# xiangli0608/Creating-2D-laser-slam-from-scratch

Measured on AMD Instinct MI355X. Metric: scan-matches/sec (1081-beam vs 2000x2000 grid), higher is better.
Workload: dtype u8

## Files before the change

### creating-2d-laser-slam-from-scratch_amd/csrc/scan_matcher.hip

```cpp
#include <algorithm>
#include <atomic>
#include <chrono>
#include <cmath>
#include <cstdlib>
#include <cstring>
#include <type_traits>
#include <vector>

#include "common.hpp"
#include "karto_math.hpp"

using namespace lslam;

#if defined(LSLAM_EXP_SERIAL_PRIO)
#define LSLAM_SERIAL_BEGIN() __builtin_amdgcn_s_setprio(3)
#define LSLAM_SERIAL_END() __builtin_amdgcn_s_setprio(0)
#else
#define LSLAM_SERIAL_BEGIN()
#define LSLAM_SERIAL_END()
#endif

namespace {

LSLAM_STAMP_TABLE(g_sm_stamps)
// ... 140 lines not shown
  };
  auto cell_y = [&](int j) {
    double y = start_y + (uint32_t)j * pc.res_y;
    double npy = center[1] + y;
    return world_to_grid(npy, g.off_y, g.scale) + g.border;
  };
  const int stx0 = pc.nx > 1 ? cell_x(1) - cell_x(0) : want_step;
  const int sty0 = pc.ny > 1 ? cell_y(1) - cell_y(0) : want_step;
  bool out_of_range = false, uneven_x = false, uneven_y = false;
  Lattice& L = lat[s];
  for (int i = lane; i < kMaxLattice; i += 64) {
    int cx = 0, cy = 0;
    if (i < pc.nx) {
      cx = cell_x(i);
      out_of_range |= cx < 0 || cx >= g.width;
      if (i >= 1) uneven_x |= cx - cell_x(i - 1) != stx0;
    }
    if (i < pc.ny) {
      cy = cell_y(i);
      out_of_range |= cy < 0 || cy >= g.height;
      if (i >= 1) uneven_y |= cy - cell_y(i - 1) != sty0;
    }
    L.gx[i] = cx;
    L.gy[i] = cy;
  }
  for (int a = lane; a < pc.na; a += 64) {
    const double angle = (center[2] - pc.ang_off) + (uint32_t)a * pc.ang_res;
    cossin[(size_t)s * kMaxAngles + a] = make_double2(cos(angle), sin(angle));
  }
  const int status = __any(out_of_range) ? LSLAM_ERR_INDEX_OUT_OF_RANGE : 0;
  const int stx = __any(uneven_x) ? 0 : stx0, sty = __any(uneven_y) ? 0 : sty0;
  if (lane == 0) {
    L.center[0] = center[0]; L.center[1] = center[1]; L.center[2] = center[2];
    L.step_x = stx;
    L.step_y = sty;
    L.status = status;
    L.active = active;
  }
}

__global__ void __launch_bounds__(64)
k_pass_setup(int S, Geom g, PassCfg pc, const double* __restrict__ poses, const CoarseOut* __restrict__ coarse,
             Lattice* __restrict__ lat, double2* __restrict__ cossin, int want_step) {
  const int s = blockIdx.x;
  if (s >= S) return;
  double center[3];
  int active = 1;
  if (pc.mode == 0) {
    center[0] = poses[3 * s]; center[1] = poses[3 * s + 1]; center[2] = poses[3 * s + 2];
  } else if (pc.mode == 1) {
    center[0] = poses[3 * s]; center[1] = poses[3 * s + 1]; center[2] = poses[3 * s + 2];
    active = coarse[s].expand && coarse[s].status == 0;
  } else {
    center[0] = coarse[s].mean[0]; center[1] = coarse[s].mean[1]; center[2] = coarse[s].mean[2];
    active = coarse[s].status == 0;
  }
  pass_setup_wave(s, threadIdx.x, g, pc, center, active, lat, cossin, want_step);
}

__global__ void __launch_bounds__(256)
k_deinterleave(const uint8_t* __restrict__ grid, uint8_t* __restrict__ f0, uint8_t* __restrict__ f1, int n8) {
  int t = blockIdx.x * blockDim.x + threadIdx.x;
  if (t >= n8) return;
  uint2 v = ((const uint2*)grid)[t];
  uint32_t e = (v.x & 0xFFu) | ((v.x >> 8) & 0xFF00u) | ((v.y & 0xFFu) << 16) | ((v.y << 8) & 0xFF000000u);
  uint32_t o = ((v.x >> 8) & 0xFFu) | ((v.x >> 16) & 0xFF00u) | ((v.y << 8) & 0xFF0000u) | (v.y & 0xFF000000u);
  ((uint32_t*)f0)[t] = e;
  ((uint32_t*)f1)[t] = o;
}

__global__ void __launch_bounds__(256)
k_tile_planes(const uint8_t* __restrict__ grid, int stride, int data_size, uint32_t* __restrict__ tiles,
              int tile_tx, int tile_rows) {
  const size_t d = (size_t)blockIdx.x * blockDim.x + threadIdx.x;
  const size_t per_class = (size_t)tile_tx * tile_rows * 8;
  if (d >= 4 * per_class) return;
  const int cls = (int)(d / per_class);
  const size_t rem = d - (size_t)cls * per_class;
  const int c4 = (int)(rem & 7);
  const size_t t = rem >> 3;
  const int row = (int)(t % tile_rows), tx = (int)(t / tile_rows);
  const int q = cls >> 1, ry = cls & 1;
  const long long y = (long long)(2 * row + ry) - kTileYOff;
  const long long m = y * (stride / 2) + 16 * tx + 4 * c4;
  uint32_t v = 0;
#pragma unroll
  for (int k = 0; k < 4; k++) {
    const long long idx = 2 * (m + k) + q;
    if (m + k >= 0 && idx < data_size) v |= (uint32_t)grid[idx] << (8 * k);
  }
  tiles[kTilePad / 4 + d] = v;
}

constexpr int kOccWinMax = 63;

__global__ void __launch_bounds__(256)
k_nonzero_bits(const uint8_t* __restrict__ grid, int data_size, uint32_t* __restrict__ nz, int n_words) {
  int w = blockIdx.x * blockDim.x + threadIdx.x;
  if (w >= n_words) return;
  uint32_t bits = 0;
  const long long f0 = (long long)w * 32;
  if (f0 + 32 <= data_size) {
    const uint4* p = (const uint4*)(grid + f0);
    uint4 a = p[0], b = p[1];
    const uint32_t v[8] = {a.x, a.y, a.z, a.w, b.x, b.y, b.z, b.w};
#pragma unroll
    for (int k = 0; k < 8; k++) {
      uint32_t d = v[k];
      bits |= ((d & 0xFFu) ? 1u : 0u) << (4 * k);
      bits |= ((d & 0xFF00u) ? 1u : 0u) << (4 * k + 1);
      bits |= ((d & 0xFF0000u) ? 1u : 0u) << (4 * k + 2);
      bits |= ((d & 0xFF000000u) ? 1u : 0u) << (4 * k + 3);
    }
  } else {
    for (int k = 0; k < 32; k++)
      if (f0 + k < data_size && grid[f0 + k] != 0) bits |= 1u << k;
  }
  nz[w] = bits;
}

__global__ void __launch_bounds__(256)
k_row_occupancy(const uint32_t* __restrict__ nz, int n_words, int stride, int height, int win,
                uint32_t* __restrict__ occ_t, int words_per_half) {
  int x = blockIdx.x * blockDim.x + threadIdx.x;
  int wq = blockIdx.y;
  if (x >= stride || wq >= 2 * words_per_half) return;
  const int E = wq / words_per_half, w2 = wq - E * words_per_half;
  const unsigned long long wmask = (1ull << win) - 1ull;
  uint32_t bits = 0;
  for (int b = 0; b < 32; b++) {
    int y = 2 * (w2 * 32 + b) + E - 1;
    if (y > height) break;
    long long f = (long long)x + (long long)y * stride;
    long long w0 = f >> 5;
    int sh = (int)(f & 31);
    unsigned long long lo = 0, hi = 0;
    if (w0 >= 0 && w0 < n_words) lo = nz[w0];
    if (w0 + 1 >= 0 && w0 + 1 < n_words) lo |= (unsigned long long)nz[w0 + 1] << 32;
    if (w0 + 2 >= 0 && w0 + 2 < n_words) hi = nz[w0 + 2];
    unsigned long long window = (lo >> sh) | (sh ? (hi << (64 - sh)) : 0ull);
    if (window & wmask) bits |= 1u << b;
  }
  occ_t[(size_t)x * (2 * words_per_half) + wq] = bits;
}

__global__ void __launch_bounds__(256)
k_occ_pairs(const uint32_t* __restrict__ occ_t, int stride, int words_per_half, uint2* __restrict__ pairs) {
  const int x = blockIdx.x * blockDim.x + threadIdx.x;
  const int ew = blockIdx.y;
  if (x >= stride) return;
  const int w = ew % words_per_half, E = ew / words_per_half;
  const uint32_t* col = occ_t + (size_t)x * (2 * words_per_half) + ew;
  pairs[((size_t)w * stride + x) * 2 + E] = make_uint2(col[0], w + 1 < words_per_half ? col[1] : 0u);
}

__device__ __forceinline__ uint32_t wave_sum(uint32_t v) {
  v += (uint32_t)__builtin_amdgcn_mov_dpp((int)v, 0xB1, 0xF, 0xF, true);
  v += (uint32_t)__builtin_amdgcn_mov_dpp((int)v, 0x4E, 0xF, 0xF, true);
  v += (uint32_t)__builtin_amdgcn_mov_dpp((int)v, 0x141, 0xF, 0xF, true);
  v += (uint32_t)__builtin_amdgcn_mov_dpp((int)v, 0x140, 0xF, 0xF, true);
  return (uint32_t)__builtin_amdgcn_readlane((int)v, 0) + (uint32_t)__builtin_amdgcn_readlane((int)v, 16) +
         (uint32_t)__builtin_amdgcn_readlane((int)v, 32) + (uint32_t)__builtin_amdgcn_readlane((int)v, 48);
}

constexpr int kPatchDw = 1536;
__device__ __forceinline__ uint32_t wave_min_u32(uint32_t v) {
  v = min(v, (uint32_t)__builtin_amdgcn_mov_dpp((int)v, 0xB1, 0xF, 0xF, true));
  v = min(v, (uint32_t)__builtin_amdgcn_mov_dpp((int)v, 0x4E, 0xF, 0xF, true));
  v = min(v, (uint32_t)__builtin_amdgcn_mov_dpp((int)v, 0x141, 0xF, 0xF, true));
  v = min(v, (uint32_t)__builtin_amdgcn_mov_dpp((int)v, 0x140, 0xF, 0xF, true));
  return min(min((uint32_t)__builtin_amdgcn_readlane((int)v, 0), (uint32_t)__builtin_amdgcn_readlane((int)v, 16)),
             min((uint32_t)__builtin_amdgcn_readlane((int)v, 32), (uint32_t)__builtin_amdgcn_readlane((int)v, 48)));
}
__device__ __forceinline__ uint32_t wave_max_u32(uint32_t v) { return ~wave_min_u32(~v); }
__device__ __forceinline__ void first_valid_min(int* s_first, bool valid, int i) {
  const unsigned long long m = __ballot(valid);
  if (m && (int)(threadIdx.x & 63) == __ffsll((long long)m) - 1) atomicMin(s_first, i);
}

constexpr int kRowsQueue = 256;
struct RowsLds {
  uint32_t (*red)[8];
  int2* queue;
  uint16_t* ambq;
  uint32_t (*patch)[kPatchDw];
  unsigned long long* ambm;
};
template <bool SOLO>
__device__ __forceinline__ void wsync() {
  if constexpr (SOLO) {
    __syncthreads();
  } else {
    __builtin_amdgcn_fence(__ATOMIC_ACQ_REL, "wavefront");
    __builtin_amdgcn_wave_barrier();
  }
}

template <int NXD, int NYC, bool TILED, bool STATS, bool LDSB, bool SOLO, bool OUT_LDS = !SOLO>
__device__ __forceinline__ void resp_rows_wave(
    const int s, const int a, const int slice, const uint8_t* __restrict__ src0, const uint8_t* __restrict__ src1, int step,
    int limit, const Geom& g, const PassCfg& pc, const Lattice* __restrict__ lat, const double2* __restrict__ cossin,
    const double2* __restrict__ local, int32_t* __restrict__ resp, size_t resp_stride, int beam_slices,
    const uint2* __restrict__ occ_t, int occ_wpc, int tile_rows, uint32_t tile_class_bytes,
    unsigned long long* __restrict__ stats, const RowsLds lds, int32_t* lds_out) {
  constexpr int NW = NXD * NYC * 2;
  constexpr bool EST = TILED;
  constexpr int kQueue = kRowsQueue;
  static_assert(NYC <= 16 && 2 * (NYC - 1) < 32, "row mask / occupancy window width");
  static_assert(SOLO || (!STATS && !LDSB), "multi-wave blocks run the production variants only");
  static_assert(!(SOLO && OUT_LDS), "a lone wave writes its numerators to global memory");
  uint32_t (*const red)[8] = lds.red;
  int2* const queue = lds.queue;
  [[maybe_unused]] uint16_t* const ambq = lds.ambq;
  [[maybe_unused]] uint32_t (*const patch)[kPatchDw] = lds.patch;
  [[maybe_unused]] unsigned long long* const ambm = lds.ambm;
  LSLAM_PHASE_CLOCK(pck);
  const Lattice& L = lat[s];
  if (!L.active || L.status != 0 || L.step_x != step || L.step_y != step) return;

  const double2 cs = cossin[(size_t)s * kMaxAngles + a];
  const double cosine = cs.x, sine = cs.y;
  auto uniform = [](float v) { return __int_as_float(__builtin_amdgcn_readfirstlane(__float_as_int(v))); };
  const float cos_sc = uniform((float)cosine * (float)g.scale), sin_sc = uniform((float)sine * (float)g.scale);
  const int X0 = L.gx[0], Y0 = L.gy[0];
  const double2* lp = local + (size_t)s * g.n_beams;
  const int ncand = pc.nx * pc.ny;
  const int shift = step == 2 ? 1 : 0;
  const int bstride = 64 * beam_slices;
  const uint8_t* zbase = TILED ? src0 : src0 - kRowZero;
  const uint32_t plane_delta = TILED ? 0u : (uint32_t)(src1 - src0);
  const uint32_t strip_bytes = (uint32_t)tile_rows * 32u;
  [[maybe_unused]] const int occ_wph = occ_wpc >> 1;

  LSLAM_PHASE_MARK(pck, 0);
  for (int j0 = 0; j0 < pc.ny; j0 += NYC) {
#if defined(LSLAM_EXP_NO_PEEL)
    constexpr bool PEEL = false;
#else
    constexpr bool PEEL = EST;
#endif
    uint32_t acc[NYC][NXD][2];
    if constexpr (!PEEL) {
#pragma unroll
      for (int j = 0; j < NYC; j++)
#pragma unroll
        for (int k = 0; k < NXD; k++) acc[j][k][0] = acc[j][k][1] = 0u;
    }
    uint32_t all_lanes = ~0u;
    asm volatile("" : "+s"(all_lanes));
    const int lane = (int)__builtin_amdgcn_mbcnt_hi(all_lanes, __builtin_amdgcn_mbcnt_lo(all_lanes, 0u));

    auto drain_as = [&](auto first_drain, int head, int cnt) {
      constexpr bool FIRST = decltype(first_drain)::value;
      const int2 e = lane < cnt ? queue[(head + lane) & (kQueue - 1)] : make_int2(0, 0);
      const uint32_t sh = (uint32_t)e.x & 3u;
      const uint32_t sel_e = 0x0C020C00u + sh * 0x00010001u;
      const uint32_t sel_o = 0x0C030C01u + sh * 0x00010001u;
      uint32_t wv[NYC][NXD + 1];
      if constexpr (TILED) {
        const uint32_t xa = (uint32_t)e.x & 0x7FFCu, yy = (uint32_t)e.x >> 16;
        const uint32_t base_off = (uint32_t)kTilePad + (((uint32_t)e.x >> 15) & 1u) * 2u * tile_class_bytes +
                                  (yy & 1u) * tile_class_bytes + (xa >> 4) * strip_bytes + (yy >> 1) * 32u +
                                  (xa & 15u);
#pragma unroll
        for (int j = 0; j < NYC; j++) {
          const uint32_t off = base_off & (uint32_t)__builtin_amdgcn_sbfe(e.y, j, 1);
          __builtin_memcpy(wv[j], __builtin_assume_aligned(zbase + (size_t)off + 32 * j, 4), 4 * (NXD + 1));
        }
      } else {
        bool staged = false;
        if constexpr (LDSB) {
          const uint32_t rowmask = (uint32_t)e.y & ((1u << NYC) - 1u);
          const bool on = lane < cnt && rowmask != 0u && e.x >= 0;
          const uint32_t cur0 = ((uint32_t)e.x & ~3u) + (uint32_t)kRowZero;
          const uint32_t ry = cur0 / (uint32_t)g.stride, cx = cur0 - ry * (uint32_t)g.stride;
          const bool p1 = e.y < 0;
          const bool bad = lane < cnt && rowmask != 0u && e.x < 0;
          uint32_t W[2], Hh[2], cmin[2], rmin[2];
          bool fit = !__any(bad);
#pragma unroll
          for (int q = 0; q < 2; q++) {
            const bool mine = on && (p1 == (q == 1));
            cmin[q] = wave_min_u32(mine ? cx : 0xFFFFFFFFu);
            rmin[q] = wave_min_u32(mine ? ry : 0xFFFFFFFFu);
            const uint32_t cmax = wave_max_u32(mine ? cx + 4u * (NXD + 1) : 0u), rmax = wave_max_u32(mine ? ry + NYC : 0u);
            W[q] = cmax > cmin[q] ? (cmax - cmin[q]) >> 2 : 0u;
            Hh[q] = rmax > rmin[q] ? rmax - rmin[q] : 0u;
            fit = fit && W[q] * Hh[q] <= (uint32_t)kPatchDw && W[q] < 65536u && Hh[q] < 65536u;
          }
          if constexpr (STATS)
            if (lane == 0 && stats) atomicAdd(&stats[fit ? 5 : 6], 1ull);
          if (fit) {
            staged = true;
            const uint32_t limit_bytes = (uint32_t)limit + (uint32_t)kRowZero;
#pragma unroll
            for (int q = 0; q < 2; q++) {
              const uint32_t total = W[q] * Hh[q];
              if (total == 0u) continue;
              const uint32_t inv = 0xFFFFFFFFu / W[q] + 1u;
              for (uint32_t idx = (uint32_t)lane; idx < total; idx += 64u) {
                const uint32_t r = __umulhi(idx, inv), c = idx - r * W[q];
                const uint32_t off = (rmin[q] + r) * (uint32_t)g.stride + cmin[q] + 4u * c;
                uint32_t v = 0u;
                if (off + 4u <= limit_bytes + 64u) v = *(const uint32_t*)(zbase + (size_t)off + (q ? plane_delta : 0u));
                patch[q][idx] = v;
              }
// ... 277 lines not shown
        const double2 p = p_next;
        p_next = lp[min(b + bstride, g.n_beams - 1)];
        const bool valid = (int)(b < g.n_beams) & (int)!isnan(p.x) & (int)!isnan(p.y);
        if constexpr (STATS) st_beams += valid ? 1u : 0u;
        int gx = 0, gy = 0;
        bool small = true;
        if (valid) exact_cell(p, gx, gy, small);
        emit(std::false_type{}, b, valid, small, gx, gy, 0, false, true, 0, 0);
      }
    }
    if (qcount > 0) drain(qhead, qcount);
    wsync<SOLO>();
    LSLAM_PHASE_MARK(pck, 1);
    if constexpr (STATS) {
      const uint32_t t0 = wave_sum(st_rows), t1 = wave_sum(st_live), t2 = wave_sum(st_beams), t3 = wave_sum(st_queued);
      if (lane == 0 && stats) {
        atomicAdd(&stats[0], (unsigned long long)t0);
        atomicAdd(&stats[1], (unsigned long long)t1);
        atomicAdd(&stats[2], (unsigned long long)t2);
        atomicAdd(&stats[3], (unsigned long long)t3);
      }
    }

#pragma unroll
    for (int j = 0; j < NYC; j++)
#pragma unroll
      for (int k = 0; k < NXD; k++)
#pragma unroll
        for (int q = 0; q < 2; q++) {
          uint32_t v = acc[j][k][q];
          v += (uint32_t)__builtin_amdgcn_mov_dpp((int)v, 0xB1, 0xF, 0xF, true);
          v += (uint32_t)__builtin_amdgcn_mov_dpp((int)v, 0x4E, 0xF, 0xF, true);
#if defined(LSLAM_EXP_NO_FUSED_DPP)
          v += (uint32_t)__builtin_amdgcn_mov_dpp((int)v, 0x141, 0xF, 0xF, true);
#else
          asm("s_nop 1\n\tv_add_u32_dpp %0, %0, %0 row_half_mirror row_mask:0xf bank_mask:0xf bound_ctrl:1" : "+v"(v));
#endif
          if ((lane & 7) == 0) red[(j * NXD + k) * 2 + q][lane >> 3] = v;
        }
    wsync<SOLO>();
    for (int idx = lane; idx < NW; idx += 64) {
      uint32_t lo = 0, hi = 0;
#pragma unroll
      for (int k = 0; k < 8; k++) {
        const uint32_t v = red[idx][k];
        lo += v & 0xFFFFu;
        hi += v >> 16;
      }
      const int par2 = idx & 1, jk = idx >> 1;
      const int j = j0 + jk / NXD, i = 4 * (jk % NXD) + par2;
      if (j < pc.ny) {
        if constexpr (OUT_LDS) {
          int32_t* o = lds_out + a * ncand + j * pc.nx + i;
          if (i < pc.nx) o[0] = (int32_t)lo;
          if (i + 2 < pc.nx) o[2] = (int32_t)hi;
        } else {
          int32_t* o = resp + (size_t)s * resp_stride + (size_t)a * ncand + (size_t)j * pc.nx + i;
          if (beam_slices == 1) {
            if (i < pc.nx) o[0] = (int32_t)lo;
            if (i + 2 < pc.nx) o[2] = (int32_t)hi;
          } else {
            if (i < pc.nx) atomicAdd(o, (int32_t)lo);
            if (i + 2 < pc.nx) atomicAdd(o + 2, (int32_t)hi);
          }
        }
      }
    }
    wsync<SOLO>();
    LSLAM_PHASE_MARK(pck, 2);
  }
  if constexpr (SOLO) LSLAM_PHASE_FLUSH(pck, g_sm_stamps, 5, (unsigned)blockIdx.x, (threadIdx.x & 63) == 0);
}

template <int NXD, int NYC, bool TILED, bool STATS = false, bool LDSB = false>
__global__ void __launch_bounds__(64) __attribute__((amdgpu_waves_per_eu(4, 8)))
k_resp_rows(const uint8_t* __restrict__ src0, const uint8_t* __restrict__ src1, int step, int limit, Geom g,
            PassCfg pc, const Lattice* __restrict__ lat, const double2* __restrict__ cossin,
            const double2* __restrict__ local, int32_t* __restrict__ resp, size_t resp_stride, int beam_slices,
            int S, const uint2* __restrict__ occ_t, int occ_wpc, int tile_rows, uint32_t tile_class_bytes,
            unsigned long long* __restrict__ stats) {
  constexpr int NW = NXD * NYC * 2;
  __shared__ __align__(16) uint32_t red[NW][8];
  __shared__ int2 queue[kRowsQueue];
  __shared__ uint16_t ambq[TILED ? 64 * kMaxBeamsPerLane : 1];
  __shared__ uint32_t patch[LDSB ? 2 : 1][LDSB ? kPatchDw : 1];
  int w = blockIdx.x;
  const int slice = w % beam_slices;
  w /= beam_slices;
  const int xcd = w & 7, r = w >> 3;
  const int s = (r / pc.na) * 8 + xcd;
  const int a = r % pc.na;
  if (s >= S) return;
  resp_rows_wave<NXD, NYC, TILED, STATS, LDSB, true>(s, a, slice, src0, src1, step, limit, g, pc, lat, cossin, local, resp,
                                                     resp_stride, beam_slices, occ_t, occ_wpc, tile_rows, tile_class_bytes,
                                                     stats, RowsLds{red, queue, ambq, (uint32_t (*)[kPatchDw])patch, nullptr},
                                                     nullptr);
}

template <int NXD>
constexpr int rows_wave_area() {
  return (NXD == 3 ? 3 * 11 * 2 * 8 * 4 : 4 * 8 * 2 * 8 * 4) > kRowsQueue * 8
             ? (NXD == 3 ? 3 * 11 * 2 * 8 * 4 : 4 * 8 * 2 * 8 * 4) + kMaxBeamsPerLane * 8
             : kRowsQueue * 8 + kMaxBeamsPerLane * 8;
}
template <int NXD, int NYC, int WAVES>
__global__ void __launch_bounds__(64 * WAVES) __attribute__((amdgpu_waves_per_eu(4, 8)))
k_resp_rows_mw(const uint8_t* __restrict__ ptiles, int limit, Geom g, PassCfg pc, const Lattice* __restrict__ lat,
               const double2* __restrict__ cossin, const double2* __restrict__ local, int32_t* __restrict__ resp,
               size_t resp_stride, int S, const uint2* __restrict__ occ_t, int occ_wpc, int tile_rows,
               uint32_t tile_class_bytes) {
  constexpr int kArea = rows_wave_area<NXD>();
  __shared__ __align__(16) unsigned char areas[WAVES * kArea];
  const int wave = (int)threadIdx.x >> 6;
  const int groups = (pc.na + WAVES - 1) / WAVES;
  const int w = blockIdx.x;
  const int xcd = w & 7, r = w >> 3;
  const int s = (r / groups) * 8 + xcd;
  const int a = (r % groups) * WAVES + wave;
  if (s >= S || a >= pc.na) return;
  unsigned char* wa = areas + wave * kArea;
  const RowsLds lds{(uint32_t (*)[8])wa, (int2*)wa, nullptr, nullptr, (unsigned long long*)(wa + (kArea - kMaxBeamsPerLane * 8))};
  resp_rows_wave<NXD, NYC, true, false, false, false, false>(s, a, 0, ptiles, ptiles, 2, limit, g, pc, lat, cossin, local, resp,
                                                             resp_stride, 1, occ_t, occ_wpc, tile_rows, tile_class_bytes,
                                                             (unsigned long long*)nullptr, lds, (int32_t*)nullptr);
}

__host__ __device__ __forceinline__ size_t tile4_slot(int ux, int uy, int cols4) {
  return ((size_t)((uy >> 1) * cols4 + (ux >> 2)) << 3) | (size_t)(((uy & 1) << 2) | (ux & 3));
}
constexpr int kTileYPad = 4;

__global__ void __launch_bounds__(256)
k_tile4(const uint8_t* __restrict__ grid, int stride, int data_size, uint4* __restrict__ tiles, int tile_cols,
        int tile_rows) {
  const int ux = blockIdx.x * blockDim.x + threadIdx.x, uy = blockIdx.y;
  if (ux >= tile_cols || uy >= tile_rows) return;
  const long long idx0 = (long long)(2 * uy - kTileYPad) * stride + 2 * ux;
  uint32_t w[4];
#pragma unroll
  for (int r = 0; r < 4; r++) {
    const long long i = idx0 + (long long)r * stride;
    uint32_t lo = 0, hi = 0;
    if (i >= 0 && i < data_size) lo = *reinterpret_cast<const uint16_t*>(grid + i);
    if (i + 2 >= 0 && i + 2 < data_size) hi = *reinterpret_cast<const uint16_t*>(grid + i + 2);
    w[r] = lo | (hi << 16);
  }
  tiles[tile4_slot(ux, uy, (tile_cols + 3) / 4)] = make_uint4(w[0], w[1], w[2], w[3]);
}

#if !defined(LSLAM_TUNE_TILE3_MIN)
#define LSLAM_TUNE_TILE3_MIN 1536
#endif
constexpr int kTile3ManyAngles = 3, kTile3ManyMinScans = LSLAM_TUNE_TILE3_MIN;
template <int kTile3Angles>
__device__ __forceinline__ void resp_tile3_wave(const int s, const int a0, const int lane, const uint4* __restrict__ tiles,
                                                int tile_cols, const Geom& g, const PassCfg& pc,
                                                const Lattice* __restrict__ lat, const double2* __restrict__ cossin,
                                                const double2* __restrict__ local, int32_t* r_scan) {
  const Lattice& L = lat[s];
  if (!L.active || L.status != 0 || L.step_x != 1 || L.step_y != 1) return;

  double cosine[kTile3Angles], sine[kTile3Angles];
  float cos_sc[kTile3Angles], sin_sc[kTile3Angles];
  bool angle_on[kTile3Angles];
#pragma unroll
  for (int q = 0; q < kTile3Angles; q++) {
    angle_on[q] = a0 + q < pc.na;
    const double2 cs = cossin[(size_t)s * kMaxAngles + min(a0 + q, pc.na - 1)];
    cosine[q] = cs.x, sine[q] = cs.y;
    cos_sc[q] = (float)cs.x * (float)g.scale, sin_sc[q] = (float)cs.y * (float)g.scale;
  }
  const int X0 = L.gx[0], Y0 = L.gy[0];
  const int B0 = X0 + Y0 * g.stride;
  const int cols4 = (tile_cols + 3) / 4;
  const double2* lp = local + (size_t)s * g.n_beams;
  uint32_t e0[kTile3Angles], e1[kTile3Angles], e2[kTile3Angles], o01[kTile3Angles], o2[kTile3Angles];
#pragma unroll
  for (int q = 0; q < kTile3Angles; q++) e0[q] = e1[q] = e2[q] = o01[q] = o2[q] = 0u;
  auto block_of = [&](const double2& p, float x32, float y32, int q, uint32_t& off, uint32_t& dx) {
    const float fx = __builtin_fmaf(cos_sc[q], x32, -(sin_sc[q] * y32)), fy = __builtin_fmaf(sin_sc[q], x32, cos_sc[q] * y32);
    const float rx = __builtin_rintf(fx), ry = __builtin_rintf(fy);
    const float reach = fabsf(fx) + fabsf(fy);
    const float lim = (0.5f - 1e-6f) - reach * (14.2f / 16777216.0f);
    int gx = (int)rx, gy = (int)ry;
    bool small = true;
    double vx = 0.0, vy = 0.0;
    if (!((int)(fabsf(fx - rx) < lim) & (int)(fabsf(fy - ry) < lim) & (int)(reach < 32000.0f))) {
      const double ox = cosine[q] * p.x - sine[q] * p.y, oy = sine[q] * p.x + cosine[q] * p.y;
      vx = ((ox + g.off_x) - g.off_x) * g.scale, vy = ((oy + g.off_y) - g.off_y) * g.scale;
      const double ax = fabs(vx) + 0.5, ay = fabs(vy) + 0.5;
      gx = (int)copysign(ax, vx), gy = (int)copysign(ay, vy);
      small = fmax(ax, ay) < 32768.0;
    }
    int x, y;
    bool ok;
    if (small) {
      x = X0 + gx, y = Y0 + gy;
      if ((uint32_t)x >= (uint32_t)g.stride) {
        const int base = B0 + gx + __mul24(gy, g.stride);
        y = base >= 0 ? base / g.stride : -((-base + g.stride - 1) / g.stride);
        x = base - y * g.stride;
      }
      ok = y >= -3 && y < g.height;
    } else {
      const int gxl = kround_i32(vx), gyl = kround_i32(vy);
      const long long base = (long long)B0 + (int)(gxl + gyl * g.stride);
      const long long yl = base >= 0 ? base / g.stride : -((-base + g.stride - 1) / g.stride);
      ok = yl >= -3 && yl < g.height;
      y = ok ? (int)yl : 0;
      x = ok ? (int)(base - yl * g.stride) : 0;
    }
    off = (uint32_t)tile4_slot(x >> 1, (y + kTileYPad) >> 1, cols4) * 16u + ((uint32_t)y & 1u) * 4u;
    dx = (uint32_t)x & 1u;
    return ok;
  };
  double2 p = lp[min(lane, g.n_beams - 1)];
  for (int b = lane; b < g.n_beams; b += 64) {
    const double2 pn = lp[min(b + 64, g.n_beams - 1)];
    if (!isnan(p.x)) {
      const float x32 = (float)p.x, y32 = (float)p.y;
      uint32_t off[kTile3Angles], dx[kTile3Angles], rr[kTile3Angles][3];
      bool ok[kTile3Angles];
#pragma unroll
      for (int q = 0; q < kTile3Angles; q++) ok[q] = block_of(p, x32, y32, q, off[q], dx[q]) && angle_on[q];
#pragma unroll
      for (int q = 0; q < kTile3Angles; q++) {
        rr[q][0] = rr[q][1] = rr[q][2] = 0u;
        if (ok[q]) __builtin_memcpy(rr[q], __builtin_assume_aligned((const uint8_t*)tiles + off[q], 4), 12);
      }
#pragma unroll
      for (int q = 0; q < kTile3Angles; q++) {
        const uint32_t r0 = rr[q][0], r1 = rr[q][1], r2 = rr[q][2];
        const uint32_t sel_e = 0x0C020C00u + dx[q] * 0x00010001u;
        const uint32_t sel_o = 0x0C050C01u + dx[q] * 0x00010001u;
        e0[q] += __builtin_amdgcn_perm(r0, r0, sel_e);
        e1[q] += __builtin_amdgcn_perm(r1, r1, sel_e);
        e2[q] += __builtin_amdgcn_perm(r2, r2, sel_e);
        o01[q] += __builtin_amdgcn_perm(r1, r0, sel_o);
        o2[q] += __builtin_amdgcn_perm(r2, r2, 0x0C0C0C01u + dx[q]);
      }
    }
    p = pn;
  }
#pragma unroll
  for (int q = 0; q < kTile3Angles; q++) {
    uint32_t tot[9];
    tot[0] = wave_sum(e0[q] & 0xFFFFu), tot[1] = wave_sum(o01[q] & 0xFFFFu), tot[2] = wave_sum(e0[q] >> 16);
    tot[3] = wave_sum(e1[q] & 0xFFFFu), tot[4] = wave_sum(o01[q] >> 16), tot[5] = wave_sum(e1[q] >> 16);
    tot[6] = wave_sum(e2[q] & 0xFFFFu), tot[7] = wave_sum(o2[q]), tot[8] = wave_sum(e2[q] >> 16);
    uint32_t mine = 0;
#pragma unroll
    for (int c = 0; c < 9; c++)
      if (lane == c) mine = tot[c];
    if (lane < 9 && angle_on[q]) r_scan[(a0 + q) * 9 + lane] = (int32_t)mine;
  }
}

template <int kTile3Angles>
__global__ void __launch_bounds__(64)
k_resp_tile3(const uint4* __restrict__ tiles, int tile_cols, Geom g, PassCfg pc, const Lattice* __restrict__ lat,
             const double2* __restrict__ cossin, const double2* __restrict__ local, int32_t* __restrict__ resp, size_t resp_stride, int S) {
  const int w = blockIdx.x;
  const int xcd = w & 7, r = w >> 3;
  const int pairs = (pc.na + kTile3Angles - 1) / kTile3Angles;
  const int s = (r / pairs) * 8 + xcd;
  const int a0 = (r % pairs) * kTile3Angles;
  if (s >= S) return;
  resp_tile3_wave<kTile3Angles>(s, a0, (int)threadIdx.x, tiles, tile_cols, g, pc, lat, cossin, local, resp + (size_t)s * resp_stride);
}

constexpr int kPosChunk = 16;
#if !defined(LSLAM_TUNE_REDUCE_NARROW_MIN)
#define LSLAM_TUNE_REDUCE_NARROW_MIN 2048
#endif
constexpr int kReduceNarrowMinScans = LSLAM_TUNE_REDUCE_NARROW_MIN;
__device__ __forceinline__ void generic_item(const uint8_t* __restrict__ grid, const Geom& g, const PassCfg& pc,
                                             const Lattice& L, const double2* __restrict__ lp, int32_t* r, int a,
                                             int c, int lane) {
  const int np = pc.nx * pc.ny;
  const double angle = (L.center[2] - pc.ang_off) + (uint32_t)a * pc.ang_res;
  const double cosine = cos(angle), sine = sin(angle);
  int pos[kPosChunk];
#pragma unroll
  for (int q = 0; q < kPosChunk; q++) {
    int f = c * kPosChunk + q;
    pos[q] = f < np ? L.gx[f % pc.nx] + L.gy[f / pc.nx] * g.stride : -1;
  }
  int32_t acc[kPosChunk];
#pragma unroll
  for (int q = 0; q < kPosChunk; q++) acc[q] = 0;
  for (int b = lane; b < g.n_beams; b += 64) {
    double2 p = lp[b];
    if (isnan(p.x)) continue;
    int t = lookup_offset(p.x, p.y, cosine, sine, g.off_x, g.off_y, g.scale, g.stride);
#pragma unroll
    for (int q = 0; q < kPosChunk; q++) {
      long long idx = (long long)pos[q] + t;
      if (pos[q] >= 0 && idx >= 0 && idx < g.data_size) acc[q] += grid[idx];
    }
  }
#pragma unroll
  for (int q = 0; q < kPosChunk; q++) {
    int v = acc[q];
    for (int o = 32; o > 0; o >>= 1) v += __shfl_xor(v, o);
    int f = c * kPosChunk + q;
    if (lane == 0 && f < np) r[(size_t)a * np + f] = v;
  }
}

__global__ void __launch_bounds__(64)
k_resp_generic(const uint8_t* __restrict__ grid, Geom g, PassCfg pc, const Lattice* __restrict__ lat,
               const double2* __restrict__ local, int32_t* __restrict__ resp, size_t resp_stride, int S) {
  const int chunks = (pc.nx * pc.ny + kPosChunk - 1) / kPosChunk;
  const int per_scan = pc.na * chunks;
  const long long total = (long long)S * per_scan;
  for (long long w = blockIdx.x; w < total; w += gridDim.x) {
    const int s = (int)(w / per_scan), rem = (int)(w % per_scan);
    const Lattice& L = lat[s];
    if (!L.active || L.status != 0) continue;
    generic_item(grid, g, pc, L, local + (size_t)s * g.n_beams, resp + (size_t)s * resp_stride, rem / chunks,
                 rem % chunks, threadIdx.x);
  }
}

__device__ __forceinline__ void block_generic_fallback(const uint8_t* __restrict__ grid, const Geom& g,
                                                       const PassCfg& pc, const Lattice& L,
                                                       const double2* __restrict__ lp, int32_t* r, int fb_step,
                                                       int tid, int nthreads) {
  if (fb_step == 0 || (L.step_x == fb_step && L.step_y == fb_step)) return;
  const int chunks = (pc.nx * pc.ny + kPosChunk - 1) / kPosChunk;
  const int per_scan = pc.na * chunks;
  for (int w = tid >> 6; w < per_scan; w += nthreads >> 6) generic_item(grid, g, pc, L, lp, r, w / chunks, w % chunks, tid & 63);
  __syncthreads();
}

struct Cand {
  double x, y, angle;
};

__device__ __forceinline__ Cand cand_of(int k, const PassCfg& pc, const double* center) {
  int a = k % pc.na, c = k / pc.na;
  int xi = c % pc.nx, yi = c / pc.nx;
  Cand cd;
  cd.x = -pc.off_x + (uint32_t)xi * pc.res_x;
  cd.y = -pc.off_y + (uint32_t)yi * pc.res_y;
  cd.angle = (center[2] - pc.ang_off) + (uint32_t)a * pc.ang_res;
  return cd;
}

__device__ __forceinline__ double penalized(int32_t sum, const Cand& cd, const double* center, int n_beams,
                                            const SearchCfg& sc) {
  double r = response_of_sum(sum, n_beams, sc);
  if (sc.do_penalize && !double_equal(r, 0.0)) {
    double sd = ksq(cd.x) + ksq(cd.y);
    double dp = 1.0 - (kDistPenaltyGain * sd / sc.dvp);
    dp = dp > sc.min_dp ? dp : sc.min_dp;
    double sad = ksq(cd.angle - center[2]);
    double ap = 1.0 - (kAnglePenaltyGain * sad / sc.avp);
    ap = ap > sc.min_ap ? ap : sc.min_ap;
    r *= (dp * ap);
  }
  return r;
}

__device__ __forceinline__ double block_max(double v, double* sh, int tid, int nthreads) {
#pragma unroll
  for (int m = 1; m < 64; m <<= 1) {
    const double o = __shfl_xor(v, m);
    v = v > o ? v : o;
  }
  if ((tid & 63) == 0) sh[tid >> 6] = v;
  __syncthreads();
  double r = sh[0];
  for (int w = 1; w < (nthreads >> 6); w++) r = r > sh[w] ? r : sh[w];
  __syncthreads();
  return r;
}

__device__ int tie_average(const uint32_t* mask, int total, const PassCfg& pc, const double* center,
                           double* avg) {
  double ax = 0, ay = 0, tx = 0, ty = 0;
  int cnt = 0;
  int words = (total + 31) / 32;
  for (int wd = 0; wd < words; wd++) {
    uint32_t m = mask[wd];
    while (m) {
      int bit = __ffs(m) - 1;
      m &= m - 1;
      int k = wd * 32 + bit;
      Cand cd = cand_of(k, pc, center);
      double h = normalize_angle(cd.angle);
      ax += center[0] + cd.x;
      ay += center[1] + cd.y;
      double sn, cs;
      sincos(h, &sn, &cs);
      tx += cs;
      ty += sn;
      cnt++;
    }
  }
  if (cnt == 0) return 0;
  ax /= cnt; ay /= cnt; tx /= cnt; ty /= cnt;
  avg[0] = ax; avg[1] = ay; avg[2] = atan2(ty, tx);
  return cnt;
}

template <bool CACHE>
__global__ void __launch_bounds__(256)
k_reduce_coarse(Geom g, PassCfg pc, SearchCfg sc, const Lattice* __restrict__ lat,
                int32_t* resp, size_t resp_stride, CoarseOut* __restrict__ out,
                int use_expansion, int pass_index, const uint8_t* __restrict__ grid,
                const double2* __restrict__ local, int fb_step) {
  extern __shared__ __align__(16) unsigned char smem[];
  __shared__ double sh[256];
  const int s = blockIdx.x, tid = threadIdx.x;
  const Lattice& L = lat[s];
  if (!L.active) return;
  if (L.status != 0) {
    if (tid == 0) { out[s].status = L.status; out[s].expand = 0; out[s].best = 0.0; }
    return;
  }
// ... 995 lines not shown
  for (int a = tid; a < kMaxAngles; a += NT) asum[a] = 0;
  LSLAM_PHASE_MARK(pck, 0);
  const double best = block_max(lm, sh, tid, NT);
  LSLAM_PHASE_MARK(pck, 1);
#pragma unroll
  for (int i = 0; i < kKeep; i++) {
    const int k = tid + NT * i;
    if (k < total && double_equal(mine[i], best)) atomicOr(&mask[k >> 5], 1u << (k & 31));
  }
  for (int k = tid + NT * kKeep; k < total; k += NT)
    if (double_equal(value(k), best)) atomicOr(&mask[k >> 5], 1u << (k & 31));
  __syncthreads();
  if (tid == 0) {
    LSLAM_SERIAL_BEGIN();
    double avg[3] = {0, 0, 0};
    int st = 0;
    if (tie_average(mask, total, pc, center, avg) == 0) st = LSLAM_ERR_NO_BEST_POSE;
    int pos = 0;
    if (st == 0) {
      int gx = world_to_grid(avg[0], g.off_x, g.scale) + g.border;
      int gy = world_to_grid(avg[1], g.off_y, g.scale) + g.border;
      if (gx < 0 || gx >= g.width || gy < 0 || gy >= g.height) st = LSLAM_ERR_INDEX_OUT_OF_RANGE;
      pos = gx + gy * g.stride;
    }
    s_avg[0] = avg[0]; s_avg[1] = avg[1]; s_avg[2] = avg[2];
    s_best = best;
    s_status = st;
    s_pos = pos;
    LSLAM_SERIAL_END();
  }
  __syncthreads();
  LSLAM_PHASE_MARK(pck, 2);
  if (s_status == 0) {
    int hit = -1;
    for (int yi = 0, c = 0; yi < pc.ny; yi++) {
      const int row = L.gy[yi] * g.stride;
      for (int xi = 0; xi < pc.nx; xi++, c++)
        if (L.gx[xi] + row == s_pos) hit = c;
    }
    if (hit >= 0) {
      for (int a = tid; a < pc.na; a += NT) asum[a] = r[a * ncand + hit];
    } else {
      const double2* lp = local + (size_t)s * g.n_beams;
      const int pos = s_pos;
      for (int a = 0; a < pc.na; a++) {
        double angle = (center[2] - pc.ang_off) + (uint32_t)a * pc.ang_res;
        double cosine = cos(angle), sine = sin(angle);
        int32_t part = 0;
        for (int b = tid; b < g.n_beams; b += NT) {
          double2 p = lp[b];
          if (isnan(p.x)) continue;
          int t = lookup_offset(p.x, p.y, cosine, sine, g.off_x, g.off_y, g.scale, g.stride);
          long long idx = (long long)pos + t;
          if (idx >= 0 && idx < g.data_size) part += grid[idx];
        }
        for (int o = 32; o > 0; o >>= 1) part += __shfl_xor(part, o);
        if ((tid & 63) == 0) atomicAdd(&asum[a], part);
      }
    }
  }
  __syncthreads();
  LSLAM_PHASE_MARK(pck, 3);
  LSLAM_PHASE_FLUSH(pck, g_sm_stamps, 4, (unsigned)(s * (NT >> 6) + (tid >> 6)), (tid & 63) == 0 && tid != 0);
  if (tid != 0) return;
  LSLAM_SERIAL_BEGIN();
  lslam_match_result res;
  memset(&res, 0, sizeof res);
  res.flags = co.flags;
  res.status = s_status;
  if (s_status == 0) {
    double bestAngle = normalize_angle_difference(s_avg[2], center[2]);
    double norm = 0.0, acc = 0.0;
    double start = center[2] - pc.ang_off;
    for (int a = 0; a < pc.na; a++) {
      double angle = start + (uint32_t)a * pc.ang_res;
      double rr = response_of_sum(asum[a], g.n_beams, sc);
      if (rr >= (s_best - 0.1)) {
        norm += rr;
        acc += (ksq(angle - bestAngle) * rr);
      }
    }
    if (norm > kTol) {
      if (acc < kTol) acc = ksq(pc.ang_res);
      acc /= norm;
    } else {
      acc = 1000 * ksq(pc.ang_res);
    }
    for (int i = 0; i < 9; i++) res.covariance[i] = co.cov[i];
    res.covariance[8] = acc;
    res.pose[0] = s_avg[0]; res.pose[1] = s_avg[1]; res.pose[2] = s_avg[2];
    res.response = s_best > 1.0 ? 1.0 : s_best;
  }
  out[s] = res;
  signal_done();
  LSLAM_PHASE_MARK(pck, 4);
  LSLAM_PHASE_FLUSH(pck, g_sm_stamps, 4, (unsigned)(s * (NT >> 6)), true);
}

template <int NT>
__global__ void __launch_bounds__(NT)
k_reduce_fine(const uint8_t* __restrict__ grid, Geom g, PassCfg pc, SearchCfg sc,
              const Lattice* __restrict__ lat, int32_t* resp, size_t resp_stride,
              const double2* __restrict__ local, const CoarseOut* __restrict__ coarse,
              lslam_match_result* __restrict__ out, int do_refine, int fb_step, int* done_flag, int done_ticket) {
  extern __shared__ __align__(16) unsigned char smem[];
  reduce_fine_block<NT>((int)blockIdx.x, (int)threadIdx.x, grid, g, pc, sc, lat, resp + (size_t)blockIdx.x * resp_stride, local,
                        coarse, out, do_refine, fb_step, done_flag, done_ticket, smem);
}

constexpr int kStepFineAngles = 4;
template <int NXD>
constexpr int step_wave_area() { return rows_wave_area<NXD>(); }
struct StepGrid {
  const uint8_t* ptiles;
  const uint2* occ;
  const uint4* tiles4;
  const uint8_t* grid;
  int limit, occ_wpc, ptile_rows, tile4_cols;
  uint32_t ptile_class_bytes;
};
template <int NXD, int NYC, int WAVES, typename RT>
__global__ void __launch_bounds__(64 * WAVES) __attribute__((amdgpu_waves_per_eu(4, 8)))
k_match_step(const RT* __restrict__ ranges, int stride, const double* __restrict__ poses, Geom g, PassCfg pc, PassCfg pf,
             SearchCfg sc, StepGrid v, Lattice* lat, double2* cossin, double2* local, CoarseOut* coarse,
             lslam_match_result* __restrict__ out, int parts, uint32_t phase_off, int32_t* dbg_coarse, int32_t* dbg_fine,
             size_t dbg_stride) {
  constexpr int NT = 64 * WAVES;
  constexpr int kArea = step_wave_area<NXD>();
  extern __shared__ __align__(16) unsigned char smem[];
  const int s = blockIdx.x, tid = threadIdx.x, wave = tid >> 6, lane = tid & 63;
  int32_t* const num = (int32_t*)smem;
  unsigned char* const phase = smem + phase_off;

  scan_prep_block(ranges, stride, poses[3 * s], poses[3 * s + 1], poses[3 * s + 2], g, local, (double2*)nullptr, pc, lat, cossin, 2,
                  0, 1, s);
  __syncthreads();
  {
    unsigned char* wa = phase + wave * kArea;
    const RowsLds lds{(uint32_t (*)[8])wa, (int2*)wa, nullptr, nullptr,
                      (unsigned long long*)(wa + (kArea - kMaxBeamsPerLane * 8))};
    for (int a = wave; a < pc.na; a += WAVES)
      resp_rows_wave<NXD, NYC, true, false, false, false>(s, a, 0, v.ptiles, v.ptiles, 2, v.limit, g, pc, lat, cossin, local,
                                                          (int32_t*)nullptr, 0, 1, v.occ, v.occ_wpc, v.ptile_rows,
                                                          v.ptile_class_bytes, (unsigned long long*)nullptr, lds, num);
  }
  __syncthreads();
  reduce_coarse_lds_block<NT>(s, tid, g, pc, sc, lat, num, coarse, 0, 0, v.grid, local, 2, pf, cossin, 1, 0, parts, phase);
  __syncthreads();
  if (dbg_coarse) {
    for (int i = tid, n = pc.nx * pc.ny * pc.na; i < n; i += NT) dbg_coarse[(size_t)s * dbg_stride + i] = num[i];
    __syncthreads();
  }
  for (int a0 = wave * kStepFineAngles; a0 < pf.na; a0 += WAVES * kStepFineAngles)
    resp_tile3_wave<kStepFineAngles>(s, a0, lane, v.tiles4, v.tile4_cols, g, pf, lat, cossin, local, num);
  __syncthreads();
  reduce_fine_block<NT>(s, tid, v.grid, g, pf, sc, lat, num, local, coarse, out, 1, 1, (int*)nullptr, 0, phase);
  if (dbg_fine) {
    __syncthreads();
    for (int i = tid, n = pf.nx * pf.ny * pf.na; i < n; i += NT) dbg_fine[(size_t)s * dbg_stride + i] = num[i];
  }
}

struct LoneSync {
  unsigned c_done, fine_ready, f_done, timeouts, pad[4];
};
constexpr int kLoneRing = 16;
__device__ __forceinline__ unsigned lone_peek(unsigned* w) {
  unsigned expected = 0xFFFFFFFFu;
  __hip_atomic_compare_exchange_strong(w, &expected, 0xFFFFFFFFu, __ATOMIC_RELAXED, __ATOMIC_RELAXED, __HIP_MEMORY_SCOPE_AGENT);
  return expected;
}
__device__ __forceinline__ bool lone_wait(unsigned* w) {
  for (int i = 0; i < (1 << 15); i++) {
    if (lone_peek(w) != 0u) return true;
    __builtin_amdgcn_s_sleep(2);
  }
  return false;
}
#if defined(LSLAM_EXP_LONE_FULL_FENCES)
#define LONE_ARRIVE_FENCE() __threadfence()
#define LONE_ACQUIRE() __threadfence()
#define LONE_RELEASE() __threadfence()
#else
#define LONE_ARRIVE_FENCE() asm volatile("s_waitcnt vmcnt(0)" ::: "memory")
#define LONE_ACQUIRE() __builtin_amdgcn_fence(__ATOMIC_ACQUIRE, "agent")
#define LONE_RELEASE() __builtin_amdgcn_fence(__ATOMIC_RELEASE, "agent")
#endif
template <int NXD, int NYC, int WAVES, int TW>
__global__ void __launch_bounds__(64 * WAVES)
k_match_lone(const uint8_t* sub0, const uint8_t* sub1, const uint8_t* grid, Geom g, PassCfg pc, PassCfg pf, SearchCfg sc,
             Lattice* lat, double2* cossin, double2* local, int32_t* resp, CoarseOut* coarse, lslam_match_result* out,
             const uint2* occ, int occ_wpc, int c_slices, int f_slices, int parts, LoneSync* ring, unsigned seq,
             int* done_flag, int done_ticket) {
  constexpr int NT = 64 * WAVES;
  constexpr int kArea = rows_wave_area<NXD>();
  extern __shared__ __align__(16) unsigned char smem[];
  __shared__ int s_last;
  const int tid = threadIdx.x, wave = tid >> 6;
  LoneSync* const sy = ring + (seq % kLoneRing);
  const int nwaves = (int)gridDim.x * TW, w = (int)blockIdx.x * TW + wave;
  LSLAM_PHASE_CLOCK(pck);

  if (wave < TW) {
    unsigned char* wa = smem + wave * kArea;
    const RowsLds lds{(uint32_t (*)[8])wa, (int2*)wa, nullptr, nullptr, nullptr};
    for (int t = w; t < pc.na * c_slices; t += nwaves)
      resp_rows_wave<NXD, NYC, false, false, false, false, false>(0, t / c_slices, t % c_slices, sub0, sub1, 2, g.data_size / 2, g, pc,
                                                                  lat, cossin, local, resp, 0, c_slices, occ, occ_wpc, 0, 0u,
                                                                  (unsigned long long*)nullptr, lds, (int32_t*)nullptr);
  }
  asm volatile("s_waitcnt vmcnt(0)" ::: "memory");
  LSLAM_PHASE_MARK(pck, 0);
  __syncthreads();
  if (tid == 0) {
    LONE_ARRIVE_FENCE();
    s_last = __hip_atomic_fetch_add(&sy->c_done, 1u, __ATOMIC_RELAXED, __HIP_MEMORY_SCOPE_AGENT) == gridDim.x - 1u;
  }
  __syncthreads();
  LSLAM_PHASE_MARK(pck, 1);
  if (s_last) {
    LONE_ACQUIRE();
    reduce_coarse_lds_block<NT>(0, tid, g, pc, sc, lat, resp, coarse, 0, 0, grid, local, 2, pf, cossin, 1, pf.nx * pf.ny * pf.na,
                                parts, smem);
    LONE_RELEASE();
    __syncthreads();
    if (tid == 0) __hip_atomic_fetch_add(&sy->fine_ready, 1u, __ATOMIC_RELAXED, __HIP_MEMORY_SCOPE_AGENT);
  } else {
    if (tid == 0 && !lone_wait(&sy->fine_ready)) __hip_atomic_fetch_add(&sy->timeouts, 1u, __ATOMIC_RELAXED, __HIP_MEMORY_SCOPE_AGENT);
    __syncthreads();
    LONE_ACQUIRE();
  }
  LSLAM_PHASE_MARK(pck, 2);
  if (wave < TW) {
    unsigned char* wa = smem + wave * kArea;
    const RowsLds lds{(uint32_t (*)[8])wa, (int2*)wa, nullptr, nullptr, nullptr};
    for (int t = w; t < pf.na * f_slices; t += nwaves)
      resp_rows_wave<1, 4, false, false, false, false, false>(0, t / f_slices, t % f_slices, grid, grid, 1, g.data_size, g, pf, lat,
                                                              cossin, local, resp, 0, f_slices, (const uint2*)nullptr, occ_wpc, 0, 0u,
                                                              (unsigned long long*)nullptr, lds, (int32_t*)nullptr);
  }
  asm volatile("s_waitcnt vmcnt(0)" ::: "memory");
  LSLAM_PHASE_MARK(pck, 3);
  __syncthreads();
  if (tid == 0) {
    LONE_ARRIVE_FENCE();
    s_last = __hip_atomic_fetch_add(&sy->f_done, 1u, __ATOMIC_RELAXED, __HIP_MEMORY_SCOPE_AGENT) == gridDim.x - 1u;
  }
  __syncthreads();
  LSLAM_PHASE_MARK(pck, 4);
  LSLAM_PHASE_FLUSH(pck, g_sm_stamps, 7, (unsigned)blockIdx.x, tid == 0);
  if (!s_last) return;
  LONE_ACQUIRE();
  const bool timed_out = lone_peek(&sy->timeouts) != 0u;
  reduce_fine_block<NT>(0, tid, grid, g, pf, sc, lat, resp, local, coarse, out, 1, 1, timed_out ? (int*)nullptr : done_flag,
                        done_ticket, smem);
  if (tid < (int)(sizeof(LoneSync) / 4)) ((unsigned*)(ring + ((seq + kLoneRing / 2) % kLoneRing)))[tid] = 0u;
  if (timed_out) {
    __syncthreads();
    if (tid == 0) {
      out[0].status = LSLAM_ERR_HIP;
      if (done_flag) {
        __threadfence_system();
        *(volatile int*)done_flag = done_ticket;
      }
    }
  }
}

__global__ void k_result_no_readings(int S, const double* poses, double coarse_ang_res,
                                     lslam_match_result* out) {
  int s = blockIdx.x * blockDim.x + threadIdx.x;
  if (s >= S) return;
  lslam_match_result r;
  memset(&r, 0, sizeof r);
  r.pose[0] = poses[3 * s]; r.pose[1] = poses[3 * s + 1]; r.pose[2] = poses[3 * s + 2];
  r.covariance[0] = kMaxVariance; r.covariance[4] = kMaxVariance;
  r.covariance[8] = 4 * ksq(coarse_ang_res);
  out[s] = r;
}

struct RebuildExtras {
  double pose[3];
  double* pose_dst;
  int32_t* zero;
  int zero_words;
  const double* ranges_src;
  double* ranges_dst;
  int n_ranges;
  const int* anchor_ring;
  const int* slot_list;
  const double* prep_ranges;
  double2* prep_local;
  Lattice* prep_lat;
  double2* prep_cossin;
  PassCfg prep_pc;
  Geom prep_g;
  int clear_blocks;
};
__global__ void __launch_bounds__(256)
k_rebuild_begin(uint4* __restrict__ grid16, size_t n16, RebuildExtras x) {
  if (x.prep_ranges && (int)blockIdx.x >= x.clear_blocks) {
    scan_prep_block(x.prep_ranges, x.prep_g.n_beams, x.pose[0], x.pose[1], x.pose[2], x.prep_g, x.prep_local,
                    (double2*)nullptr, x.prep_pc, x.prep_lat, x.prep_cossin, 2, (int)blockIdx.x - x.clear_blocks,
                    (int)gridDim.x - x.clear_blocks, 0);
    return;
  }
  const size_t i = (size_t)blockIdx.x * blockDim.x + threadIdx.x;
// ... 2100 lines not shown
```

Before: 7.269 million.

## Reduce tile3 per-lane counters through LDS and use magic-number rounding

```diff
diff --git a/creating-2d-laser-slam-from-scratch_amd/csrc/scan_matcher.hip b/creating-2d-laser-slam-from-scratch_amd/csrc/scan_matcher.hip
--- a/creating-2d-laser-slam-from-scratch_amd/csrc/scan_matcher.hip
+++ b/creating-2d-laser-slam-from-scratch_amd/csrc/scan_matcher.hip
@@ -316,6 +316,12 @@
   const int w = ew % words_per_half, E = ew / words_per_half;
   const uint32_t* col = occ_t + (size_t)x * (2 * words_per_half) + ew;
   pairs[((size_t)w * stride + x) * 2 + E] = make_uint2(col[0], w + 1 < words_per_half ? col[1] : 0u);
+}
+
+__device__ __forceinline__ float round_fast(float f, int& i) {
+  const float t = f + 0x1.8p23f;
+  i = (int)(__float_as_uint(t) - 0x4B400000u);
+  return t - 0x1.8p23f;
 }
 
 __device__ __forceinline__ uint32_t wave_sum(uint32_t v) {
@@ -899,11 +905,12 @@
 #define LSLAM_TUNE_TILE3_MIN 1536
 #endif
 constexpr int kTile3ManyAngles = 3, kTile3ManyMinScans = LSLAM_TUNE_TILE3_MIN;
+constexpr int kTile3RedPitch = 68;
 template <int kTile3Angles>
 __device__ __forceinline__ void resp_tile3_wave(const int s, const int a0, const int lane, const uint4* __restrict__ tiles,
                                                 int tile_cols, const Geom& g, const PassCfg& pc,
                                                 const Lattice* __restrict__ lat, const double2* __restrict__ cossin,
-                                                const double2* __restrict__ local, int32_t* r_scan) {
+                                                const double2* __restrict__ local, int32_t* r_scan, uint32_t* red) {
   const Lattice& L = lat[s];
   if (!L.active || L.status != 0 || L.step_x != 1 || L.step_y != 1) return;
 
@@ -916,6 +923,8 @@
     const double2 cs = cossin[(size_t)s * kMaxAngles + min(a0 + q, pc.na - 1)];
     cosine[q] = cs.x, sine[q] = cs.y;
     cos_sc[q] = (float)cs.x * (float)g.scale, sin_sc[q] = (float)cs.y * (float)g.scale;
+    asm("" : "+v"(cos_sc[q]));
+    asm("" : "+v"(sin_sc[q]));
   }
   const int X0 = L.gx[0], Y0 = L.gy[0];
   const int B0 = X0 + Y0 * g.stride;
@@ -926,10 +935,10 @@
   for (int q = 0; q < kTile3Angles; q++) e0[q] = e1[q] = e2[q] = o01[q] = o2[q] = 0u;
   auto block_of = [&](const double2& p, float x32, float y32, int q, uint32_t& off, uint32_t& dx) {
     const float fx = __builtin_fmaf(cos_sc[q], x32, -(sin_sc[q] * y32)), fy = __builtin_fmaf(sin_sc[q], x32, cos_sc[q] * y32);
-    const float rx = __builtin_rintf(fx), ry = __builtin_rintf(fy);
+    int gx, gy;
+    const float rx = round_fast(fx, gx), ry = round_fast(fy, gy);
     const float reach = fabsf(fx) + fabsf(fy);
     const float lim = (0.5f - 1e-6f) - reach * (14.2f / 16777216.0f);
-    int gx = (int)rx, gy = (int)ry;
     bool small = true;
     double vx = 0.0, vy = 0.0;
     if (!((int)(fabsf(fx - rx) < lim) & (int)(fabsf(fy - ry) < lim) & (int)(reach < 32000.0f))) {
@@ -989,6 +998,40 @@
     }
     p = pn;
   }
+  if constexpr (5 * kTile3Angles <= 16) {
+    constexpr int kWords = 5 * kTile3Angles;
+#pragma unroll
+    for (int q = 0; q < kTile3Angles; q++) {
+      red[(5 * q + 0) * kTile3RedPitch + lane] = e0[q];
+      red[(5 * q + 1) * kTile3RedPitch + lane] = e1[q];
+      red[(5 * q + 2) * kTile3RedPitch + lane] = e2[q];
+      red[(5 * q + 3) * kTile3RedPitch + lane] = o01[q];
+      red[(5 * q + 4) * kTile3RedPitch + lane] = o2[q];
+    }
+    wsync<true>();
+    const int w = lane >> 2, qt = lane & 3;
+    uint32_t lo = 0u, hi = 0u;
+    if (w < kWords) {
+      const uint4* src = reinterpret_cast<const uint4*>(red + w * kTile3RedPitch + qt * 16);
+#pragma unroll
+      for (int i = 0; i < 4; i++) {
+        const uint4 v = src[i];
+        lo += (v.x & 0xFFFFu) + (v.y & 0xFFFFu) + (v.z & 0xFFFFu) + (v.w & 0xFFFFu);
+        hi += (v.x >> 16) + (v.y >> 16) + (v.z >> 16) + (v.w >> 16);
+      }
+    }
+    lo += (uint32_t)__builtin_amdgcn_mov_dpp((int)lo, 0xB1, 0xF, 0xF, true);
+    hi += (uint32_t)__builtin_amdgcn_mov_dpp((int)hi, 0xB1, 0xF, 0xF, true);
+    lo += (uint32_t)__builtin_amdgcn_mov_dpp((int)lo, 0x4E, 0xF, 0xF, true);
+    hi += (uint32_t)__builtin_amdgcn_mov_dpp((int)hi, 0x4E, 0xF, 0xF, true);
+    const int q = w / 5, k = w - 5 * q;
+    if (qt == 0 && w < kWords && a0 + q < pc.na) {
+      int32_t* o = r_scan + (a0 + q) * 9;
+      o[(0x71630u >> (4 * k)) & 15u] = (int32_t)lo;
+      if (k != 4) o[(0x4852u >> (4 * k)) & 15u] = (int32_t)hi;
+    }
+    return;
+  }
 #pragma unroll
   for (int q = 0; q < kTile3Angles; q++) {
     uint32_t tot[9];
@@ -1004,7 +1047,7 @@
 }
 
 template <int kTile3Angles>
-__global__ void __launch_bounds__(64)
+__global__ void __launch_bounds__(64) __attribute__((amdgpu_waves_per_eu(8, 8)))
 k_resp_tile3(const uint4* __restrict__ tiles, int tile_cols, Geom g, PassCfg pc, const Lattice* __restrict__ lat,
              const double2* __restrict__ cossin, const double2* __restrict__ local, int32_t* __restrict__ resp, size_t resp_stride, int S) {
   const int w = blockIdx.x;
@@ -1013,7 +1056,9 @@
   const int s = (r / pairs) * 8 + xcd;
   const int a0 = (r % pairs) * kTile3Angles;
   if (s >= S) return;
-  resp_tile3_wave<kTile3Angles>(s, a0, (int)threadIdx.x, tiles, tile_cols, g, pc, lat, cossin, local, resp + (size_t)s * resp_stride);
+  __shared__ __align__(16) uint32_t red[5 * kTile3Angles * kTile3RedPitch];
+  resp_tile3_wave<kTile3Angles>(s, a0, (int)threadIdx.x, tiles, tile_cols, g, pc, lat, cossin, local, resp + (size_t)s * resp_stride,
+                                red);
 }
 
 constexpr int kPosChunk = 16;
@@ -2315,7 +2360,7 @@
     __syncthreads();
   }
   for (int a0 = wave * kStepFineAngles; a0 < pf.na; a0 += WAVES * kStepFineAngles)
-    resp_tile3_wave<kStepFineAngles>(s, a0, lane, v.tiles4, v.tile4_cols, g, pf, lat, cossin, local, num);
+    resp_tile3_wave<kStepFineAngles>(s, a0, lane, v.tiles4, v.tile4_cols, g, pf, lat, cossin, local, num, nullptr);
   __syncthreads();
   reduce_fine_block<NT>(s, tid, v.grid, g, pf, sc, lat, num, local, coarse, out, 1, 1, (int*)nullptr, 0, phase);
   if (dbg_fine) {
```

Result: faster. 7.358 million, median of 6 (+1.2%).
